# Nikhil-Kulkarni/RayTrace-miniapp

Measured on AMD Instinct MI355X. Metric: ray_steps_per_sec, higher is better.
Workload: dtype f32+f64

## Files before the change

### raytrace-miniapp_amd/csrc/rt_march.hip

```cpp
#pragma once
#include "rt_math.h"

#include <cfloat>

namespace rt {

enum : int { ST_IDLE = 0, ST_CELL = 1, ST_XSETUP = 2, ST_STEP = 3, ST_DONE = 4 };

typedef double f64x2 __attribute__((ext_vector_type(2)));
typedef float f32x4 __attribute__((ext_vector_type(4)));
typedef unsigned u32x4 __attribute__((ext_vector_type(4)));

__device__ __forceinline__ unsigned div_magic(unsigned x, unsigned mul, unsigned sh)
{
    return mul ? __umulhi(x, mul) >> sh : x;
}
__device__ __forceinline__ void grid_index(const DevRays &R, unsigned ridx, unsigned &i, unsigned &j, unsigned &k,
                                           unsigned &m)
{
    const unsigned ijkm = (unsigned) (R.first + (long long) ridx * R.stride);
    const unsigned q1   = div_magic(ijkm, R.div_mul[0], R.div_sh[0]);
    m                   = ijkm - q1 * (unsigned) R.ngb;
    const unsigned q2   = div_magic(q1, R.div_mul[1], R.div_sh[1]);
    k                   = q1 - q2 * (unsigned) R.nga;
    i                   = div_magic(q2, R.div_mul[2], R.div_sh[2]);
    j                   = q2 - i * (unsigned) R.ngy;
}

__device__ __forceinline__ void load_ray(const DevRays &R, unsigned ridx, rt_ray &ray, float &ta, float &tb,
                                         bool want_tan)
{
    if (R.list) {
        ray = R.list[ridx];
        if (want_tan) {
            ta = R.sxy[2 * (size_t) ridx];
            tb = R.sxy[2 * (size_t) ridx + 1];
        }
    } else {
        unsigned i, j, k, m;
        grid_index(R, ridx, i, j, k, m);
        ray.x      = (float) R.gx[i];
        ray.y      = (float) R.gy[j];
        ray.a      = (float) R.ga[k];
        ray.b      = (float) R.gb[m];
        if (want_tan) {
            ta = R.tan_a[k];
            tb = R.tan_b[m];
        }
    }
}

__device__ __attribute__((noinline)) float tan_wide(float x)
{
    if (!(fabsf(x) <= FLT_MAX))
        return x - x;
    return (float) tan((double) x);
}
__device__ __attribute__((noinline)) float atan_wide(float x)
{
    if (x != x)
        return x + x;
    if (!(fabsf(x) <= FLT_MAX))
        return copysignf(1.5707963705062866f, x);
    return (float) atan((double) x);
}

__device__ __attribute__((noinline)) float ktanf_flt32(float x, float y, int iy)
{
    const float T[13] = { 3.3333334327e-01f, 1.3333334029e-01f, 5.3968254477e-02f, 2.1869488060e-02f, 8.8632395491e-03f,
                          3.5920790397e-03f, 1.4562094584e-03f, 5.8804126456e-04f, 2.4646313977e-04f, 7.8179444245e-05f,
                          7.1407252108e-05f, -1.8558637748e-05f, 2.5907305826e-05f };
    const float pio4 = 7.8539812565e-01f, pio4lo = 3.7748947079e-08f;
    float z, r, v, w, s;
    const int hx = (int) __float_as_uint(x), ix = hx & 0x7fffffff;
    if (ix < 0x39000000) {
        if ((int) x == 0) {
            if ((ix | (iy + 1)) == 0)
                return 1.0f / fabsf(x);
            else if (iy == 1)
                return x;
            else
                return -1.0f / x;
        }
    }
    if (ix >= 0x3f2ca140) {
        if (hx < 0) {
            x = -x;
            y = -y;
        }
        z = pio4 - x;
        w = pio4lo - y;
        x = z + w;
        y = 0.0f;
        if (fabsf(x) < 0x1p-13f)
            return (1 - ((hx >> 30) & 2)) * iy * (1.0f - 2 * iy * x);
    }
    z = x * x;
    w = z * z;
    r = T[1] + w * (T[3] + w * (T[5] + w * (T[7] + w * (T[9] + w * T[11]))));
    v = z * (T[2] + w * (T[4] + w * (T[6] + w * (T[8] + w * (T[10] + w * T[12])))));
    s = z * x;
    r = y + z * (s * (r + v) + y);
    r += T[0] * s;
    w = x + r;
    if (ix >= 0x3f2ca140) {
        v = (float) iy;
        return (float) (1 - ((hx >> 30) & 2)) * (v - 2.0f * (x - (w * w / (w + v) - r)));
    }
    if (iy == 1)
        return w;
    float a, t;
    z = __uint_as_float(__float_as_uint(w) & 0xfffff000u);
    v = r - (z - x);
    t = a = -1.0f / w;
    t = __uint_as_float(__float_as_uint(t) & 0xfffff000u);
    s = 1.0f + t * z;
    return t + a * (s + t * v);
}
__device__ __attribute__((noinline)) float tanf_flt32_wide(float x)
{
    const float pio2_1 = 1.5707855225e+00f, pio2_1t = 1.0804334124e-05f, pio2_2 = 1.0804273188e-05f,
                pio2_2t = 6.0770999344e-11f;
    const int hx = (int) __float_as_uint(x), ix = hx & 0x7fffffff;
    if (ix <= 0x3f490fda)
        return ktanf_flt32(x, 0.0f, 1);
    float y0, y1, z;
    if (hx > 0) {
        z = x - pio2_1;
        if ((ix & 0xfffffff0) != 0x3fc90fd0) {
            y0 = z - pio2_1t;
            y1 = (z - y0) - pio2_1t;
        } else {
            z -= pio2_2;
            y0 = z - pio2_2t;
            y1 = (z - y0) - pio2_2t;
        }
    } else {
        z = x + pio2_1;
        if ((ix & 0xfffffff0) != 0x3fc90fd0) {
            y0 = z + pio2_1t;
            y1 = (z - y0) + pio2_1t;
        } else {
            z += pio2_2;
            y0 = z + pio2_2t;
            y1 = (z - y0) + pio2_2t;
        }
    }
    return ktanf_flt32(y0, y1, -1);
}

__device__ __forceinline__ float tanf_flt32_kernel(float x)
{
    const float ax = fabsf(x);
    if (ax < 0x1p-13f)
        return x;
    if (ax > 0.2f) {
        if (!(ax <= FLT_MAX))
            return x - x;
        return ax <= 1.375f ? tanf_flt32_wide(x) : tan_wide(x);
    }
    const float T0 = 3.3333334327e-01f, T1 = 1.3333334029e-01f, T2 = 5.3968254477e-02f, T3 = 2.1869488060e-02f,
                T4 = 8.8632395491e-03f, T5 = 3.5920790397e-03f, T6 = 1.4562094584e-03f, T7 = 5.8804126456e-04f,
                T8 = 2.4646313977e-04f, T9 = 7.8179444245e-05f, T10 = 7.1407252108e-05f, T11 = -1.8558637748e-05f,
                T12 = 2.5907305826e-05f;
    const float z = x * x;
    const float w = z * z;
    float r       = T1 + w * (T3 + w * (T5 + w * (T7 + w * (T9 + w * T11))));
    const float v = z * (T2 + w * (T4 + w * (T6 + w * (T8 + w * (T10 + w * T12)))));
    const float s = z * x;
    r             = 0.0f + z * (s * (r + v) + 0.0f);
    r += T0 * s;
    return x + r;
}

__device__ __forceinline__ float atanf_flt32_kernel(float x)
{
    const float ax = fabsf(x);
    if (ax < 0x1p-29f)
        return x;
    if (!(ax < 0.4375f))
        return atan_wide(x);
    const float A0 = 3.3333334327e-01f, A1 = -2.0000000298e-01f, A2 = 1.4285714924e-01f, A3 = -1.1111110449e-01f,
                A4 = 9.0908870101e-02f, A5 = -7.6918758452e-02f, A6 = 6.6610731184e-02f, A7 = -5.8335702866e-02f,
                A8 = 4.9768779427e-02f, A9 = -3.6531571299e-02f, A10 = 1.6285819933e-02f;
    const float z  = x * x;
    const float w  = z * z;
    const float s1 = z * (A0 + w * (A2 + w * (A4 + w * (A6 + w * (A8 + w * A10)))));
    const float s2 = w * (A1 + w * (A3 + w * (A5 + w * (A7 + w * A9))));
    return x - x * (s1 + s2);
}

extern "C" __global__ void __launch_bounds__(256) rt_seed_tab_kernel(const DevSeed sd, const DevRays R, double *sf,
                                                                     unsigned char *sin)
{
    const int n0 = R.ngx, n1 = R.ngy, n2 = R.nga, n3 = R.ngb;
    for (int t = (int) (blockIdx.x * blockDim.x + threadIdx.x); t < n0 + n1 + n2 + n3; t += (int) (gridDim.x * blockDim.x)) {
        int d           = t < n0 ? 0 : (t < n0 + n1 ? 1 : (t < n0 + n1 + n2 ? 2 : 3));
        const int i     = t - (d > 0 ? n0 : 0) - (d > 1 ? n1 : 0) - (d > 2 ? n2 : 0);
        const double *g = d == 0 ? R.gx : (d == 1 ? R.gy : (d == 2 ? R.ga : R.gb));
        const double v  = (double) (float) g[i];
        const bool in   = v >= sd.x[d][0] && v <= sd.x[d][sd.dim[d] - 1];
        sin[t]          = in ? 1 : 0;
        sf[t]           = in ? pchip_eval(sd.dim[d], sd.x[d], sd.f[d], v) : 0.0;
    }
}

__device__ __forceinline__ unsigned selftest_hash(unsigned x)
{
    x ^= x >> 16;
    x *= 0x7feb352du;
    x ^= x >> 15;
    x *= 0x846ca68bu;
    x ^= x >> 16;
    return x;
}
extern "C" __global__ void __launch_bounds__(256) rt_selftest_kernel(unsigned long long *counts)
{
    const unsigned lo = 0x3f700000u, hi = 0x3f880000u;
    const unsigned n_fast = hi - lo, n_other = 1u << 24;
    unsigned long long checked = 0, bad = 0;
    const unsigned long long tid = (unsigned long long) blockIdx.x * blockDim.x + threadIdx.x;
    const unsigned long long nth = (unsigned long long) gridDim.x * blockDim.x;
    for (unsigned long long t = tid; t < (unsigned long long) n_fast + n_other; t += nth) {
        const unsigned u = t < n_fast ? lo + (unsigned) t : (unsigned) (t - n_fast) << 8;
        float q          = __uint_as_float(u);
        const float a    = inv_norm(q);
        asm volatile("" : "+v"(q));
        const float b = 1.0f / sqrtf(q);
        checked++;
        if (__float_as_uint(a) != __float_as_uint(b) && !(a != a && b != b))
            bad++;
    }
    for (unsigned long long t = tid; t < (4ull << 23); t += nth) {
        float n       = __uint_as_float(0x3e800000u + (unsigned) t);
        const float a = fdiv_one_nr(n);
        asm volatile("" : "+v"(n));
        const float b = 1.0f / n;
        checked++;
        bad += __float_as_uint(a) != __float_as_uint(b) ? 1 : 0;
    }
    for (unsigned long long t = tid; t < (1ull << 28); t += nth) {
        const unsigned h0 = selftest_hash((unsigned) t * 2u + 1u), h1 = selftest_hash((unsigned) t * 2u + 0x9e3779b9u);
        const int ea = -84 + (int) (h0 % 84u), eb = -78 + (int) (h1 % 122u);
        if (ea - eb >= 96 || eb - ea >= 96 || ea - eb < -120)
            continue;
        float x = __uint_as_float(((unsigned) (ea + 127) << 23) | (selftest_hash(h0) & 0x7fffffu));
        float y = __uint_as_float(((unsigned) (eb + 127) << 23) | (selftest_hash(h1) & 0x7fffffu));
        const float a = fdiv_nr(x, y);
        asm volatile("" : "+v"(x), "+v"(y));
        const float b = x / y;
        checked++;
        bad += __float_as_uint(a) != __float_as_uint(b) ? 1 : 0;
    }
    if (tid == 0) {
        float inf = __uint_as_float(0x7f800000u), qnan = __uint_as_float(0x7fc00000u), big = 3.0e38f;
        asm volatile("" : "+v"(inf), "+v"(qnan), "+v"(big));
        const unsigned pio2 = 0x3fc90fdbu;
        const float t0 = tanf_flt32_kernel(inf), t1 = tanf_flt32_kernel(-inf), t2 = tanf_flt32_kernel(qnan), t3 = tan_wide(inf),
                    t4 = tan_wide(qnan), t5 = tanf_flt32_kernel(big);
        const float a0 = atanf_flt32_kernel(inf), a1 = atanf_flt32_kernel(-inf), a2 = atanf_flt32_kernel(qnan),
                    a3 = atanf_flt32_kernel(big), a4 = atanf_flt32_kernel(-big);
        checked += 11;
        bad += (t0 == t0) + (t1 == t1) + (t2 == t2) + (t3 == t3) + (t4 == t4) + (__float_as_uint(t5) == 0x7fc12345u);
        bad += (__float_as_uint(a0) != pio2) + (__float_as_uint(a1) != (pio2 | 0x80000000u)) + (a2 == a2) +
               (__float_as_uint(a3) != pio2) + (__float_as_uint(a4) != (pio2 | 0x80000000u));
    }
    atomicAdd(&counts[0], checked);
    atomicAdd(&counts[1], bad);
}

extern "C" __global__ void __launch_bounds__(256) rt_tan_kernel(const rt_ray *rays, unsigned long long n, float *sxy)
{
    unsigned long long i = (unsigned long long) blockIdx.x * blockDim.x + threadIdx.x;
    if (i < n) {
        rt_ray r       = rays[i];
        sxy[2 * i]     = tanf_flt32_kernel(1e-3f * r.a);
        sxy[2 * i + 1] = tanf_flt32_kernel(1e-3f * r.b);
    }
}

__device__ __forceinline__ int bisect_interval(const Interval *iv, int n, double v)
{
    int lo = 0, hi = n - 1;
    while (hi - lo != 1) {
        int mid = (hi + lo) / 2;
        if (iv[mid].hi >= v)
            hi = mid;
        else
            lo = mid;
    }
    return hi;
}
__device__ __forceinline__ int guess_interval(int n, float g0, float inv_h, float v)
{
    return (int) fminf(fmaxf((v - g0) * inv_h, 0.0f), (float) (n - 2)) + 1;
}

#ifdef RT_INSTRUMENT
__device__ unsigned short g_ray_iters[1u << 23];
#endif
#ifdef RT_WAVETIMES
__device__ unsigned long long g_wt[8];
__device__ unsigned long long g_wt_end[8192], g_wt_dry[8192];
constexpr int WT_TRACE = 64;
__device__ unsigned long long g_wt_trace[8192][WT_TRACE];
__device__ unsigned g_wt_blocks[8192][WT_TRACE][6];
#endif
struct TileList {
    unsigned *head;
    unsigned *next;
    unsigned *lnode;
    unsigned *nalloc;
    unsigned cap;
    unsigned *rem;
    unsigned *marching;
    unsigned n_waves;
    unsigned split;
    unsigned k_part;
};
constexpr unsigned TILE_NONE = 0xffffffffu;
constexpr unsigned TILE_PART_FLAG = 1u << 30, TILE_PART_SHIFT = 28, TILE_ID_MASK = (1u << TILE_PART_SHIFT) - 1u;
__device__ __forceinline__ unsigned tile_node(unsigned entry)
{
    return (entry & TILE_ID_MASK) * 4u + ((entry & TILE_PART_FLAG) ? (entry >> TILE_PART_SHIFT) & 3u : 0u);
}
#ifdef RT_WAVETIMES
__device__ unsigned long long g_wt_pub[8192][4];
__device__ unsigned long long g_wt_vm[8192];
#endif
constexpr unsigned TILE_REF_GLOBAL = 1u << 31;
__device__ __forceinline__ void tile_push(const TileList &T, unsigned tile)
{
    const unsigned id = __hip_atomic_fetch_add(T.nalloc, 1u, __ATOMIC_RELAXED, __HIP_MEMORY_SCOPE_WORKGROUP);
    unsigned old      = __hip_atomic_load(T.head, __ATOMIC_RELAXED, __HIP_MEMORY_SCOPE_WORKGROUP);
    if (id < T.cap) {
        __hip_atomic_store(&T.lnode[2u * id], tile, __ATOMIC_RELAXED, __HIP_MEMORY_SCOPE_WORKGROUP);
        for (;;) {
            __hip_atomic_store(&T.lnode[2u * id + 1u], old, __ATOMIC_RELAXED, __HIP_MEMORY_SCOPE_WORKGROUP);
            asm volatile("s_waitcnt lgkmcnt(0)" ::: "memory");
            if (__hip_atomic_compare_exchange_strong(T.head, &old, id, __ATOMIC_RELAXED, __ATOMIC_RELAXED, __HIP_MEMORY_SCOPE_WORKGROUP))
                return;
#ifdef RT_WAVETIMES
            g_wt_pub[(blockIdx.x * (blockDim.x >> 6) + (threadIdx.x >> 6)) & 8191u][2]++;
#endif
        }
    }
    tile |= TILE_REF_GLOBAL;
    for (;;) {
        __hip_atomic_store(&T.next[tile_node(tile & ~TILE_REF_GLOBAL)], old, __ATOMIC_RELAXED, __HIP_MEMORY_SCOPE_WORKGROUP);
        asm volatile("s_waitcnt vmcnt(0)" ::: "memory");
        if (__hip_atomic_compare_exchange_strong(T.head, &old, tile, __ATOMIC_RELAXED, __ATOMIC_RELAXED, __HIP_MEMORY_SCOPE_WORKGROUP))
            return;
#ifdef RT_WAVETIMES
        g_wt_pub[(blockIdx.x * (blockDim.x >> 6) + (threadIdx.x >> 6)) & 8191u][2]++;
#endif
    }
}
__device__ __forceinline__ void tile_publish(const TileList &T, unsigned tile)
{
    bool parts = T.split == 2u;
    if (T.split == 1u)
        parts = __hip_atomic_load(T.head, __ATOMIC_RELAXED, __HIP_MEMORY_SCOPE_WORKGROUP) == TILE_NONE &&
                __hip_atomic_load(T.marching, __ATOMIC_RELAXED, __HIP_MEMORY_SCOPE_WORKGROUP) * 8u <= T.n_waves;
    if (parts && T.k_part != 0u) {
        for (unsigned q = 0; q < 4u; q++)
            tile_push(T, tile | (q << TILE_PART_SHIFT) | TILE_PART_FLAG);
    } else {
        tile_push(T, tile);
    }
}
__device__ __forceinline__ unsigned tile_pop(const TileList &T)
{
    unsigned old = __hip_atomic_load(T.head, __ATOMIC_RELAXED, __HIP_MEMORY_SCOPE_WORKGROUP);
    while (old != TILE_NONE) {
        const unsigned nxt = (old & TILE_REF_GLOBAL)
                                 ? __hip_atomic_load(&T.next[tile_node(old & ~TILE_REF_GLOBAL)], __ATOMIC_RELAXED, __HIP_MEMORY_SCOPE_WORKGROUP)
                                 : __hip_atomic_load(&T.lnode[2u * old + 1u], __ATOMIC_RELAXED, __HIP_MEMORY_SCOPE_WORKGROUP);
        if (__hip_atomic_compare_exchange_strong(T.head, &old, nxt, __ATOMIC_RELAXED, __ATOMIC_RELAXED, __HIP_MEMORY_SCOPE_WORKGROUP))
            break;
    }
    if (old == TILE_NONE)
        return TILE_NONE;
    return (old & TILE_REF_GLOBAL) ? (old & ~TILE_REF_GLOBAL) : __hip_atomic_load(&T.lnode[2u * old], __ATOMIC_RELAXED, __HIP_MEMORY_SCOPE_WORKGROUP);
}

template <bool LDS_TAB> __device__ __forceinline__ void march_load_tables(const DevParams &P, unsigned char *lds_raw)
{
    if (LDS_TAB) {
        const uint4 *src = reinterpret_cast<const uint4 *>(P.blob);
        uint4 *dst       = reinterpret_cast<uint4 *>(lds_raw);
        const unsigned n16 = P.blob_bytes / 16, step = blockDim.x;
        for (unsigned i0 = threadIdx.x; i0 < n16; i0 += 8 * step) {
            uint4 v[8];
#pragma unroll
            for (int u = 0; u < 8; u++) {
                const unsigned i = i0 + (unsigned) u * step;
                v[u]             = src[i < n16 ? i : i0];
            }
#pragma unroll
            for (int u = 0; u < 8; u++) {
                const unsigned i = i0 + (unsigned) u * step;
                if (i < n16)
                    dst[i] = v[u];
            }
        }
        __syncthreads();
    }
}

template <bool LDS_TAB, bool BOUNDED, bool FUSED, int MODE = 0>
__device__ __forceinline__ void march_wave(const DevParams &P, unsigned char *lds_raw, const TileList done)
{
    const int lane        = lane_id();
    const int L           = P.L;
    const int S           = L * RT_N_SUB;
    const unsigned n_rays = P.ray_end;
    const bool backward   = MODE == 1 ? true : ((MODE == 2 || MODE == 3) ? false : P.method == 1);
    const bool use_emis   = MODE == 1 ? true : ((MODE == 2 || MODE == 4) ? false : P.use_emis != 0);
    const bool path_on    = MODE == 0 ? P.path_on != 0 : false;
    const unsigned CH     = P.chunk;
#ifndef RT_REFILL
#define RT_REFILL 8
#endif
    const int REFILL      = RT_REFILL;

    const unsigned char *tab = LDS_TAB ? lds_raw : P.blob;
    const BlobGain *hdr = reinterpret_cast<const BlobGain *>(tab);
    const unsigned lds_base = LDS_TAB ? (unsigned) (size_t) (__attribute__((address_space(3))) unsigned char *) lds_raw : 0u;

    static_assert(RT_N_SUB == 3, "sub-segment ends are tabulated for three sub-segments");
    float zs0 = (P.dz0 * (0.0f + 1.0f) / RT_N_SUB), zs1 = (P.dz0 * (1.0f + 1.0f) / RT_N_SUB),
          zs2 = (P.dz0 * (2.0f + 1.0f) / RT_N_SUB);
    asm volatile("" : "+v"(zs0), "+v"(zs1), "+v"(zs2));

    unsigned chunk_next = 0, chunk_end = 0;
    unsigned fetched_end = 0, slot_busy = 0, cur_slot = 0;
    unsigned cslot       = 0;
    bool more           = true;
    const unsigned n_launch_rays = n_rays - P.ray_begin;
    const unsigned n_chunks      = (n_launch_rays + CH - 1) / CH;
    unsigned shard = blockIdx.x & 7u, shards_seen_empty = 0;
    const unsigned n_main = n_chunks - (P.late_chunks < n_chunks ? P.late_chunks : 0u);
    const bool late_wave  = (unsigned) __builtin_amdgcn_readfirstlane((int) (threadIdx.x >> 6)) - P.late_first < P.late_waves;
    unsigned zone = 0;

    int st        = ST_IDLE;
    unsigned ridx = 0;
    int seg = 0, iz = 0, ii = 0;
    float z = 0.0f, z_stop = 0.0f;
    float px = 0, py = 0, pz = 0, sx = 0, sy = 0, sz = 1;
    float gacc = 0, eacc = 0;
    int cell_last = 0, sub = 0;
    unsigned char *recp = P.rec;
    unsigned lane12     = 0;
    BlobGain G    = hdr[1];
    unsigned steps = 0;
    bool escaped = false, mirror = false;
    unsigned any_bits = 0;
    int c00 = 0;
    float f00 = 1, f10 = 1, f01 = 1, f11 = 1;
    double dnx0 = 0, dnx1 = 0, dny0 = 0, dny1 = 0;
    f64x2 ix0 = { 0.0, 1.0 }, iy0 = { 0.0, 1.0 };
    f32x4 ix1 = { 1.0f, 0.0f, 0.0f, 0.0f }, iy1 = { 1.0f, 0.0f, 0.0f, 0.0f };
    float g0 = 0, E0 = 0;
    float dzrem = 0, zc = 0, path = 0;
    float rx = 0, ry = 0, rz = 0, n = 0, n0 = 0, gxn = 0, gyn = 0, lim2 = 0, dzcap = 0, hsum = 0;
    unsigned tot_steps = 0, tot_esc = 0, tot_rays = 0, tot_skip = 0;
#ifdef RT_INSTRUMENT
    Inst inst;
#endif

#if defined(RT_TIMEBLOCKS) || defined(RT_WAVEBLOCKS)
    unsigned long long tb_acc[6] = { 0, 0, 0, 0, 0, 0 }, tb_last = __builtin_readcyclecounter(), tb_iters = 0;
#endif
#ifdef RT_WAVETIMES
    const unsigned long long wt_start = __builtin_amdgcn_s_memrealtime();
    unsigned long long wt_dry = 0;
    unsigned wt_a_runs = 0, wt_b_runs = 0;
#endif
#ifdef RT_INSTRUMENT
    unsigned ray_iters = 0;
#endif
    unsigned spin = 0;
#if defined(RT_EXPRESS) || defined(RT_WAVETIMES)
    unsigned wave_iter = 0;
#endif
#ifdef RT_EXPRESS
    unsigned born = 0;
    bool old_wave = false;
    if (P.express_tail == 1u)
        __builtin_amdgcn_s_setprio(2);
#else
    constexpr bool old_wave = false;
#endif
    for (;;) {
        RT_MARK(5);
#ifdef RT_INSTRUMENT
        ray_iters += st != ST_IDLE ? 1u : 0u;
#endif
#ifdef RT_TIMEBLOCKS
        tb_iters++;
#endif
        unsigned long long idle2      = __ballot(st == ST_IDLE);
        const unsigned long long idle = idle2;
        const int n_idle              = (int) __popcll(idle);
#if defined(RT_EXPRESS) || defined(RT_WAVETIMES)
        wave_iter++;
#endif
#ifdef RT_WAVETIMES
        if ((wave_iter & 15u) == 0u) {
            const unsigned wid = blockIdx.x * (blockDim.x >> 6) + (threadIdx.x >> 6), smp = wave_iter >> 4;
            if (lane == 0 && wid < 8192u && smp < (unsigned) WT_TRACE) {
                g_wt_trace[wid][smp] = (__builtin_amdgcn_s_memrealtime() & 0xffffffffffull) | ((unsigned long long) (WAVE - n_idle) << 40) |
                                       ((unsigned long long) wt_a_runs << 48) | ((unsigned long long) wt_b_runs << 56);
                g_wt_trace[wid][0] = smp;
#ifdef RT_WAVEBLOCKS
                for (int b = 0; b < 6; b++)
                    g_wt_blocks[wid][smp][b] = (unsigned) tb_acc[b];
#endif
            }
#ifdef RT_WAVEBLOCKS
            for (int b = 0; b < 6; b++)
                tb_acc[b] = 0;
#endif
            wt_a_runs = wt_b_runs = 0;
        }
#endif
#ifdef RT_EXPRESS
        if (P.express_age != 0u && (wave_iter & 3u) == 0u) {
            const bool o = __ballot(st != ST_IDLE && wave_iter - born > P.express_age) != 0ull;
            if (o != old_wave) {
                old_wave = o;
                if (o)
                    __builtin_amdgcn_s_setprio(3);
                else
                    __builtin_amdgcn_s_setprio(0);
            }
        }
#endif
        if (!BOUNDED) {
            if (((++spin) & 0xfffu) == 0u && spin >= P.spin_limit) {
                spin = 0;
                if (st != ST_IDLE) {
                    escaped = true;
                    sx = sy = sz = 0.0f;
                    st           = ST_CELL;
                }
            }
        }
        if (more && (n_idle >= REFILL)) {
            const int rank = (int) __builtin_amdgcn_mbcnt_hi((unsigned) (idle >> 32),
                                                             __builtin_amdgcn_mbcnt_lo((unsigned) idle, 0u));
            int need = n_idle, off = 0;
            bool got = false;
            while (need > 0) {
                if (chunk_next == chunk_end && !(FUSED && chunk_next != fetched_end)) {
#ifdef RT_EXPRESS
                    if (old_wave && P.express_hold != 0u)
                        break;
#endif
                    unsigned c = 0;
#ifdef RT_MARCH_ONE_COUNTER
                    if (lane == 0)
                        c = atomicAdd(&P.ctl->next_tile[P.launch_id][0][0], 1u);
                    c = (unsigned) __builtin_amdgcn_readfirstlane((int) c);
                    shards_seen_empty = 7;
#else
                    if (lane == 0)
                        c = atomicAdd(&P.ctl->next_tile[P.launch_id][shard][zone * 8u], 1u);
                    c = (unsigned) __builtin_amdgcn_readfirstlane((int) c) * 8u + shard + zone * n_main;
#endif
                    if (c >= (zone ? n_chunks : n_main)) {
                        if (++shards_seen_empty == 8) {
                            if (zone == 0u && late_wave && n_main < n_chunks) {
                                zone              = 1u;
                                shards_seen_empty = 0;
                                continue;
                            }
                            more = false;
#ifdef RT_EXPRESS
                            if (P.express_tail == 2u)
                                __builtin_amdgcn_s_setprio(3);
#endif
#ifdef RT_WAVETIMES
                            wt_dry = __builtin_amdgcn_s_memrealtime();
#endif
                            break;
                        }
                        shard = (shard + 1) & 7u;
                        continue;
                    }
                    chunk_next = P.ray_begin + c * CH;
                    chunk_end  = (n_rays - chunk_next < CH) ? n_rays : chunk_next + CH;
                    if (FUSED) {
                        fetched_end = chunk_end;
                        chunk_end   = chunk_next;
                    }
                }
                if (FUSED && chunk_next == chunk_end) {
#ifndef RT_FUSED_PUBLISH_WAVE
                    const unsigned in_use = lane < 32 ? __hip_atomic_load(&done.rem[lane], __ATOMIC_RELAXED, __HIP_MEMORY_SCOPE_WAVEFRONT) : 1u;
                    slot_busy             = ~(unsigned) __ballot(lane < 32 && in_use == 0u);
#endif
                    const int fs = __builtin_ffs((int) ~slot_busy) - 1;
                    if (fs < 0)
                        break;
                    chunk_end = fetched_end - chunk_next < (unsigned) WAVE ? fetched_end : chunk_next + (unsigned) WAVE;
                    cur_slot  = (unsigned) fs;
                    slot_busy |= 1u << fs;
                    if (lane == 0)
                        __hip_atomic_store(&done.rem[fs], chunk_end - chunk_next, __ATOMIC_RELAXED, __HIP_MEMORY_SCOPE_WAVEFRONT);
                }
                int avail = (int) (chunk_end - chunk_next);
                int take  = avail < need ? avail : need;
                if (st == ST_IDLE && !got && rank >= off && rank < off + take) {
                    ridx = chunk_next + (unsigned) (rank - off);
                    got  = true;
                    if (FUSED)
                        cslot = cur_slot;
                }
                chunk_next += (unsigned) take;
                need -= take;
                off += take;
            }
            if (!BOUNDED && __ballot(got) != 0ull)
                spin = 0;
            if (got) {
                rt_ray ray;
                float ta = 0, tb = 0;
                load_ray(P.rays, ridx, ray, ta, tb, true);
                px = ray.x;
                py = ray.y;
                pz = 0.0f;
                sx = ta;
                sy = tb;
                sz = 1.0f;
                if (backward) {
                    sx = -sx;
                    sy = -sy;
                    sz = -sz;
                }
                renormalise(sx, sy, sz);
                const BlobGain G0 = hdr[backward ? P.N - 1 : 1];
                const float dsum  = sx + sy + sz;
                const bool wild   = ((px != px) | (py != py) | (dsum != dsum)) &
                                  !((px < G0.lo_x) | (px > G0.hi_x) | (py < G0.lo_y) | (py > G0.hi_y));
                if (path_on) {
                    float *pp = P.path + (size_t) ridx * 3 * (size_t) (S + 1) + 3 * (size_t) (backward ? S : 0);
                    pp[0]     = px;
                    pp[1]     = py;
                }
                recp      = P.rec + rec_slot_off(ridx, backward ? S - 1 : 0, P.rec_stride);
                lane12    = (ridx & 63u) * 12u;
                seg       = 0;
                iz        = 0;
                ii        = backward ? P.N - 1 : 1;
                G         = G0;
                z         = 0.0f;
                z_stop    = zs0;
                gacc      = 0.0f;
                eacc      = 0.0f;
                cell_last = 0;
                steps     = 0;
                escaped   = wild;
                sx        = wild ? 0.0f : sx;
                sy        = wild ? 0.0f : sy;
                sz        = wild ? 0.0f : sz;
                any_bits  = P.no_skip;
                sub       = 0;
                st        = ST_CELL;
#ifdef RT_EXPRESS
                born      = wave_iter;
#endif
            }
            idle2 = __ballot(st == ST_IDLE);
        }
        if (idle2 == ~0ull) {
            if (!more)
                break;
        } else {

        RT_MARK(0);
        const unsigned long long want_a = __ballot(st == ST_CELL);
        int park_at = (int) P.park;
        if (!more || old_wave || (int) P.park > 12 || REFILL > 8) {
            const int n_live = WAVE - (int) __popcll(idle2);
            const int fifth  = (n_live * 13 + 63) >> 6;
            park_at          = fifth < (int) P.park ? fifth : (int) P.park;
#ifdef RT_EXPRESS
            if (old_wave && P.express_park != 0u)
                park_at = (n_live * (int) P.express_park + 63) >> 6;
#endif
        }
        const bool do_a = (int) __popcll(want_a) >= park_at || (~(idle2 | want_a)) == 0ull;
#ifdef RT_FUSED_PUBLISH_WAVE
        bool last_of_tile = false;
#endif
#ifdef RT_WAVETIMES
        wt_a_runs += (do_a && want_a != 0ull) ? 1u : 0u;
        wt_b_runs += __ballot(st == ST_XSETUP) != 0ull ? 1u : 0u;
#endif
        if (do_a && st == ST_CELL) {
            bool in_seg        = !escaped & (z < 0.995f * z_stop);
            if (!in_seg) {
#ifndef RT_ABL_NOSTORE
                *reinterpret_cast<RecSlot *>(recp) = RecSlot{ gacc, eacc, cell_last };
#endif
                recp += backward ? -(int) REC_SLOT_ROW : (int) REC_SLOT_ROW;
                any_bits |= (__float_as_uint(gacc) | __float_as_uint(eacc)) & 0x7fffffffu;
                if (path_on) {
                    float *pp = P.path + (size_t) ridx * 3 * (size_t) (S + 1);
                    for (int zz = iz; zz < (escaped ? RT_N_SUB : iz + 1); zz++) {
                        const int idx = RT_N_SUB * (ii - 1) + (backward ? RT_N_SUB - zz - 1 : zz + 1);
                        pp[3 * idx]     = px;
                        pp[3 * idx + 1] = py;
                    }
                }
                gacc      = 0.0f;
                eacc      = 0.0f;
                cell_last = 0;
                sub++;
                const bool wrap = iz == RT_N_SUB - 1;
                const bool fin  = escaped | (sub == S);
                iz              = wrap ? 0 : iz + 1;
                z               = wrap ? 0.0f : z;
                st              = fin ? ST_DONE : ST_CELL;
                if (wrap & !fin) {
                    seg++;
                    ii = backward ? P.N - seg - 1 : seg + 1;
                    G  = hdr[ii];
                }
                z_stop = iz == 0 ? zs0 : (iz == 1 ? zs1 : zs2);
                in_seg = !fin & (z < 0.995f * z_stop);
            }
            RT_MARK(1);
            if ((st == ST_CELL) & in_seg) {
                if ((px < G.lo_x) | (px > G.hi_x) | (py < G.lo_y) | (py > G.hi_y) | (sz * sz <= 0.01f)) {
                    escaped = true;
                } else {
                    mirror              = G.mirror_y != 0;
                    const Interval *ivx = reinterpret_cast<const Interval *>(tab + G.off_ix);
                    const Interval *ivy = reinterpret_cast<const Interval *>(tab + G.off_iy);
                    f64x2 tx, ty;
                    u32x4 q00, q10, q01, q11;
                    auto gather = [&](int k1, int k2, int c) {
                        const unsigned ox = (unsigned) G.off_ix + (unsigned) k1 * (unsigned) sizeof(Interval);
                        const unsigned oy = (unsigned) G.off_iy + (unsigned) k2 * (unsigned) sizeof(Interval);
                        const unsigned oa = (unsigned) G.off_node + (unsigned) c * (unsigned) sizeof(Node);
                        const unsigned ob = oa + (unsigned) G.Nx * (unsigned) sizeof(Node);
                        if (LDS_TAB) {
                            asm volatile("ds_read_b128 %0, %10\n\t"
                                         "ds_read_b128 %1, %10 offset:16\n\t"
                                         "ds_read_b128 %2, %10 offset:32\n\t"
                                         "ds_read_b128 %3, %11\n\t"
                                         "ds_read_b128 %4, %11 offset:16\n\t"
                                         "ds_read_b128 %5, %11 offset:32\n\t"
                                         "ds_read_b128 %6, %12\n\t"
                                         "ds_read_b128 %7, %12 offset:16\n\t"
                                         "ds_read_b128 %8, %13\n\t"
                                         "ds_read_b128 %9, %13 offset:16\n\t"
                                         "s_waitcnt lgkmcnt(0)"
                                         : "=&v"(ix0), "=&v"(ix1), "=&v"(tx), "=&v"(iy0), "=&v"(iy1), "=&v"(ty), "=&v"(q00), "=&v"(q10),
                                           "=&v"(q01), "=&v"(q11)
                                         : "v"(lds_base + ox), "v"(lds_base + oy), "v"(lds_base + oa), "v"(lds_base + ob));
                        } else {
                            const unsigned char *t = tab;
                            ix0 = *reinterpret_cast<const f64x2 *>(t + ox);
                            ix1 = *reinterpret_cast<const f32x4 *>(t + ox + 16);
                            tx  = *reinterpret_cast<const f64x2 *>(t + ox + 32);
                            iy0 = *reinterpret_cast<const f64x2 *>(t + oy);
                            iy1 = *reinterpret_cast<const f32x4 *>(t + oy + 16);
                            ty  = *reinterpret_cast<const f64x2 *>(t + oy + 32);
                            q00 = *reinterpret_cast<const u32x4 *>(t + oa);
                            q10 = *reinterpret_cast<const u32x4 *>(t + oa + 16);
                            q01 = *reinterpret_cast<const u32x4 *>(t + ob);
                            q11 = *reinterpret_cast<const u32x4 *>(t + ob + 16);
                        }
                    };
                    auto node_n = [](const u32x4 &q) { return __hiloint2double((int) q.y, (int) q.x); };
                    const float ya      = mirror ? fabsf(py) : py;
                    const double pxd = (double) px, yad = (double) ya;
                    int k1     = guess_interval(G.Nx, G.x0f, G.inv_hxf, px);
                    int k2     = guess_interval(G.Ny, G.y0f, G.inv_hyf, ya);
                    c00        = (k1 - 1) + (k2 - 1) * G.Nx;
                    gather(k1, k2, c00);
                    const bool ok = ((k1 == 1) | (ix0.x < pxd)) & ((k1 == G.Nx - 1) | (tx.x >= pxd)) &
                                    ((k2 == 1) | (iy0.x < yad)) & ((k2 == G.Ny - 1) | (ty.x >= yad));
                    if (!ok) {
                        k1  = bisect_interval(ivx, G.Nx, pxd);
                        k2  = bisect_interval(ivy, G.Ny, yad);
                        c00 = (k1 - 1) + (k2 - 1) * G.Nx;
                        gather(k1, k2, c00);
                    }
                    const double n00 = node_n(q00), n10 = node_n(q10), n01 = node_n(q01), n11 = node_n(q11);
                    f00       = (float) n00;
                    f10       = (float) n10;
                    f01       = (float) n01;
                    f11       = (float) n11;
                    dnx0      = n10 - n00;
                    dnx1      = n11 - n01;
                    dny0      = n01 - n00;
                    dny1      = n11 - n10;
                    const float u = (float) div_by_recip<true>(pxd - ix0.x, tx.x - ix0.x, tx.y);
                    const float v = (float) div_by_recip<true>(yad - iy0.x, ty.x - iy0.x, ty.y);
                    g0            = lerp2(u, v, __uint_as_float(q00.z), __uint_as_float(q10.z), __uint_as_float(q01.z),
                                          __uint_as_float(q11.z));
                    E0            = 0.0f;
                    if (use_emis) {
                        E0 = lerp2(u, v, __uint_as_float(q00.w), __uint_as_float(q10.w), __uint_as_float(q01.w),
                                   __uint_as_float(q11.w));
                        E0 = E0 >= 0 ? E0 : 0.0f;
                    }
                    pz    = 0.0f;
                    zc    = 0.0f;
                    path  = 0.0f;
                    dzrem = z_stop - z;
                    if ((px > ix1.y) & (px < ix1.z) & (ya > iy1.y) & (ya < iy1.z) & (dzrem > 0.0f)) {
                        st = ST_XSETUP;
                    } else {
                        z += fabsf(pz);
                        gacc += g0 * path;
                        eacc += E0 * path;
                        cell_last = c00;
                        steps++;
                        RT_TICK(2);
                    }
                }
            }
            RT_MARK(2);
            if (st == ST_DONE) {
                unsigned fl = F_VALID;
                if (escaped)
                    fl |= F_ESCAPED;
                if (use_emis && any_bits == 0u)
                    fl |= F_SKIP;
                RecMeta m;
                m.px          = px;
                m.py          = py;
                m.sx          = sx;
                m.sy          = sy;
                m.sz          = sz;
                m.flags_steps = fl | ((unsigned) sub << REC_NDONE_SHIFT) |
                                ((steps < 0xfffffu ? steps : 0xfffffu) << REC_STEPS_SHIFT);
                unsigned char *metap = recp + (int) REC_SLOT_ROW * (backward ? sub + 1 : S - sub) + lane12;
#ifndef RT_ABL_NOMETA
                *reinterpret_cast<RecMeta *>(metap) = m;
#else
                if (m.px == 1234.5f)
                    *reinterpret_cast<RecMeta *>(metap) = m;
#endif
#ifdef RT_INSTRUMENT
                if (ridx < (1u << 23))
                    g_ray_iters[ridx] = (unsigned short) (ray_iters < 65535u ? ray_iters : 65535u);
                ray_iters = 0;
#endif
                tot_steps += steps;
                tot_esc += escaped ? 1u : 0u;
                tot_skip += (fl & F_SKIP) ? 1u : 0u;
                tot_rays++;
                st = ST_IDLE;
#ifdef RT_FUSED_PUBLISH_WAVE
                if (FUSED)
                    last_of_tile = __hip_atomic_fetch_add(&done.rem[cslot], 0xffffffffu, __ATOMIC_RELAXED, __HIP_MEMORY_SCOPE_WAVEFRONT) == 1u;
#else
                if (FUSED) {
                    if (__hip_atomic_fetch_add(&done.rem[cslot], 0xffffffffu, __ATOMIC_RELAXED, __HIP_MEMORY_SCOPE_WAVEFRONT) == 1u) {
                        asm volatile("s_waitcnt vmcnt(0)" ::: "memory");
                        tile_publish(done, ridx >> 6);
                    }
                }
#endif
            }
        }
#ifdef RT_FUSED_PUBLISH_WAVE
        if (FUSED) {
            unsigned long long lm = __ballot(last_of_tile);
            if (lm != 0ull) {
#ifdef RT_WAVETIMES
                const unsigned long long vm0 = __builtin_amdgcn_s_memrealtime();
#endif
                asm volatile("s_waitcnt vmcnt(0)" ::: "memory");
#ifdef RT_WAVETIMES
                if (lane == 0)
                    g_wt_vm[(blockIdx.x * (blockDim.x >> 6) + (threadIdx.x >> 6)) & 8191u] += __builtin_amdgcn_s_memrealtime() - vm0;
#endif
                do {
                    const int l0 = (int) __ffsll((long long) lm) - 1;
                    lm &= lm - 1ull;
#ifdef RT_WAVETIMES
                    const unsigned long long pub0 = __builtin_amdgcn_s_memrealtime();
#endif
                    if (lane == l0)
                        tile_publish(done, ridx >> 6);
#ifdef RT_WAVETIMES
                    if (lane == l0) {
                        const unsigned long long dt = __builtin_amdgcn_s_memrealtime() - pub0;
                        unsigned long long *q = g_wt_pub[(blockIdx.x * (blockDim.x >> 6) + (threadIdx.x >> 6)) & 8191u];
                        q[0] += dt;
                        q[1] += 1;
                        q[3] = dt > q[3] ? dt : q[3];
                    }
#endif
                    slot_busy &= ~(1u << (unsigned) __builtin_amdgcn_readlane((int) cslot, l0));
                } while (lm != 0ull);
            }
        }
#endif
        RT_MARK(3);
        if (st == ST_XSETUP) {
            const float ya   = mirror ? fabsf(py) : py;
            const double dwx = (double) ix1.x, dwy = (double) iy1.x;
            const double xc0 = ix0.x, yc0 = iy0.x, rwx = ix0.y, rwy = iy0.y;
            const float u    = (float) div_by_recip<true>((double) px - xc0, dwx, rwx);
            const float v    = (float) div_by_recip<true>((double) ya - yc0, dwy, rwy);
            n0  = lerp2(u, v, f00, f10, f01, f11);
            gxn = (float) (div_by_recip<true>((1.0 - (double) v) * dnx0, dwx, rwx) +
                           div_by_recip<true>((double) v * dnx1, dwx, rwx));
            gyn = (float) (div_by_recip<true>((1.0 - (double) u) * dny0, dwy, rwy) +
                           div_by_recip<true>((double) u * dny1, dwy, rwy));
            if (mirror && py < 0)
                gyn = -gyn;
            lim2  = dzrem - zc;
            dzcap = P.c_cap * lim2;
            rx    = 0.0f;
            ry    = 0.0f;
            rz    = 0.0f;
            n     = n0;
            hsum  = 0.0f;
            st    = ST_STEP;
            RT_TICK(1);
        }

        RT_MARK(4);
        if (st == ST_STEP) {
            const float lim0 = 0.1f * ix1.x, lim1 = 0.1f * iy1.x;
            bool run;
            {
                n        = n0 + rx * gxn + ry * gyn;
#ifdef RT_ABL_FASTDIV
#define RT_FDIV(a, b) ((a) * __builtin_amdgcn_rcpf(b))
#else
#define RT_FDIV(a, b) ((a) / (b))
#endif
                const float rn = BOUNDED ? fdiv_one_nr(n) : RT_FDIV(1.0f, n);
                float a0 = sx * gxn + sy * gyn + 1e-12f;
                float t  = BOUNDED ? fmaf(fmaf(-n, a0 * rn, a0), rn, a0 * rn) : div_by_recip_signed(a0, n, rn);
                float qx = div_by_recip_signed(gxn, n, rn);
                float qy = div_by_recip_signed(gyn, n, rn);
#ifndef RT_ABL_NOGUARD
                if (__ballot(fminf(fminf(fabsf(a0), fabsf(gxn)), fabsf(gyn)) < 1e-29f) != 0ull) {
#ifdef RT_INSTRUMENT
                    if (lane == (int) __ffsll((long long) __ballot(1)) - 1)
                        atomicAdd(&g_inst[6], 1ull);
#endif
                    if (fabsf(a0) < 1e-29f && a0 != 0.0f) {
                        asm volatile("" : "+v"(a0));
                        t = a0 / n;
                    }
                    if (fabsf(gxn) < 1e-29f && gxn != 0.0f) {
                        float g = gxn;
                        asm volatile("" : "+v"(g));
                        qx = g / n;
                    }
                    if (fabsf(gyn) < 1e-29f && gyn != 0.0f) {
                        float g = gyn;
                        asm volatile("" : "+v"(g));
                        qy = g / n;
                    }
                }
#endif
                float fx = qx - sx * t;
                float fy = qy - sy * t;
                float fz = -sz * t;
                float h;
                if (BOUNDED) {
                    const float h1 = fdiv_nr(P.c_h1, fabsf(t));
                    const float h2 = fdiv_nr(1.0001f * (lim2 - fabsf(rz)), fabsf(sz));
                    const float h3 = fdiv_nr(P.c_h3 * (fabsf(sx) + 5e-4f), (fabsf(fx) + 1e-8f));
                    const float h4 = fdiv_nr(P.c_h3 * (fabsf(sy) + 5e-4f), (fabsf(fy) + 1e-8f));
                    h = fmin_nan_drop(fmin_nan_drop(h1, dzcap), fmin_nan_drop(h2, fmin_nan_drop(h3, h4)));
                } else {
                    h        = RT_FDIV(P.c_h1, fabsf(t));
                    h        = h < dzcap ? h : dzcap;
                    float h2 = RT_FDIV(1.0001f * (lim2 - fabsf(rz)), fabsf(sz));
                    float h3 = RT_FDIV(P.c_h3 * (fabsf(sx) + 5e-4f), (fabsf(fx) + 1e-8f));
                    float h4 = RT_FDIV(P.c_h3 * (fabsf(sy) + 5e-4f), (fabsf(fy) + 1e-8f));
                    h        = h < h2 ? h : h2;
                    h        = h < h3 ? h : h3;
                    h        = h < h4 ? h : h4;
                }
                float ht = h * t;
                const float R3 = 1.0f / 3.0f, R6 = 1.0f / 6.0f, R12 = 1.0f / 12.0f;
                float c1 = 0.5f * h * h * (1.0f - div_by_recip<true>(ht, 3.0f, R3) + div_by_recip<true>(ht * ht, 12.0f, R12));
                rx += sx * h + c1 * fx;
                ry += sy * h + c1 * fy;
                rz += sz * h + c1 * fz;
                float c2 = h * (1.0f - 0.5f * ht + div_by_recip<true>(ht * ht, 6.0f, R6));
                sx += c2 * fx;
                sy += c2 * fy;
                sz += c2 * fz;
                renormalise(sx, sy, sz);
                hsum += h;
                RT_TICK(0);
                run = (fabsf(rx) < lim0) & (fabsf(ry) < lim1) & (fabsf(rz) < lim2) & (fabsf(n - n0) < 0.05f);
            }
            if (!run) {
                path += hsum;
                px += rx;
                py += ry;
                pz += rz;
                zc += fabsf(rz);
                const float ya = mirror ? fabsf(py) : py;
                if ((px > ix1.y) & (px < ix1.z) & (ya > iy1.y) & (ya < iy1.z) & ((double) zc < 0.999 * (double) dzrem)) {
                    st = ST_XSETUP;
                } else {
                    z += fabsf(pz);
                    gacc += g0 * path;
                    eacc += E0 * path;
                    cell_last = c00;
                    steps++;
                    RT_TICK(2);
                    st = ST_CELL;
                }
            }
        }
        }
    }
#ifdef RT_EXPRESS
    if (P.express_age != 0u || P.express_tail != 0u)
        __builtin_amdgcn_s_setprio(0);
#endif

#ifdef RT_WAVETIMES
    if (lane == 0) {
        const unsigned long long wt_end = __builtin_amdgcn_s_memrealtime();
        atomicMin(&g_wt[0], wt_start);
        atomicMax(&g_wt[1], wt_start);
        const unsigned w = atomicAdd((unsigned *) &g_wt[6], 1u);
        if (w < 8192)
            g_wt_end[w] = wt_end | ((unsigned long long) (threadIdx.x >> 6) << 56), g_wt_dry[w] = wt_dry;
    }
#endif
    {
        unsigned s = wave_sum_u32(tot_steps), e = wave_sum_u32(tot_esc);
        unsigned k = wave_sum_u32(tot_skip), r = wave_sum_u32(tot_rays);
#ifndef RT_ABL_NOTOTALS
        if (lane == 0) {
            atomicAdd(&P.ctl->cell_steps, (unsigned long long) s);
            atomicAdd(&P.ctl->n_escaped, (unsigned long long) e);
            atomicAdd(&P.ctl->n_skipped, (unsigned long long) k);
            atomicAdd(&P.ctl->n_rays, (unsigned long long) r);
        }
#else
        if (lane == 0 && s + e + k + r == 0xffffffffu)
            atomicAdd(&P.ctl->cell_steps, 1ull);
#endif
#ifdef RT_TIMEBLOCKS
        if (lane == 0) {
            for (int i = 0; i < 6; i++)
                atomicAdd(&g_inst[i], tb_acc[i]);
            atomicAdd(&g_inst[7], tb_iters);
        }
#endif
#ifdef RT_INSTRUMENT
        for (int i = 0; i < 3; i++) {
            unsigned tw = wave_sum_u32(inst.w[i]), ta = wave_sum_u32(inst.a[i]);
            if (lane == 0) {
                atomicAdd(&g_inst[2 * i], (unsigned long long) tw);
                atomicAdd(&g_inst[2 * i + 1], (unsigned long long) ta);
            }
        }
#endif
    }
}

template <bool LDS_TAB, bool BOUNDED, int MODE = 0>
__global__ void __launch_bounds__(LDS_TAB ? 1024 : 256) rt_march_kernel(const DevParams P)
{
    extern __shared__ __align__(16) unsigned char lds_raw[];
    march_load_tables<LDS_TAB>(P, lds_raw);
    march_wave<LDS_TAB, BOUNDED, false, MODE>(P, lds_raw, TileList{ nullptr, nullptr, nullptr, nullptr, 0u, nullptr, nullptr, 0u, 0u, 0u });
}

}
```

Measured before the change: 29.40 billion.

## Precompute ray start state per tile and hand it to lanes via bpermute

```diff
diff --git a/raytrace-miniapp_amd/csrc/rt_march.hip b/raytrace-miniapp_amd/csrc/rt_march.hip
--- a/raytrace-miniapp_amd/csrc/rt_march.hip
+++ b/raytrace-miniapp_amd/csrc/rt_march.hip
@@ -423,6 +423,11 @@
 #define RT_REFILL 8
 #endif
     const int REFILL      = RT_REFILL;
+#ifdef RT_NO_TILE_START
+    constexpr bool TILE_START = false;
+#else
+    constexpr bool TILE_START = FUSED;
+#endif
 
     const unsigned char *tab = LDS_TAB ? lds_raw : P.blob;
     const BlobGain *hdr = reinterpret_cast<const BlobGain *>(tab);
@@ -466,6 +471,28 @@
     float dzrem = 0, zc = 0, path = 0;
     float rx = 0, ry = 0, rz = 0, n = 0, n0 = 0, gxn = 0, gyn = 0, lim2 = 0, dzcap = 0, hsum = 0;
     unsigned tot_steps = 0, tot_esc = 0, tot_rays = 0, tot_skip = 0;
+    float bank_px = 0, bank_py = 0, bank_sx = 0, bank_sy = 0, bank_sz = 0;
+    unsigned long long bank_wild = 0ull;
+    auto start_state = [&](const unsigned r, float &qx, float &qy, float &ux, float &uy, float &uz) {
+        rt_ray ray;
+        float ta = 0, tb = 0;
+        load_ray(P.rays, r, ray, ta, tb, true);
+        qx = ray.x;
+        qy = ray.y;
+        ux = ta;
+        uy = tb;
+        uz = 1.0f;
+        if (backward) {
+            ux = -ux;
+            uy = -uy;
+            uz = -uz;
+        }
+        renormalise(ux, uy, uz);
+        const BlobGain &G0 = hdr[backward ? P.N - 1 : 1];
+        const float dsum   = ux + uy + uz;
+        return (bool) (((qx != qx) | (qy != qy) | (dsum != dsum)) &
+                       !((qx < G0.lo_x) | (qx > G0.hi_x) | (qy < G0.lo_y) | (qy > G0.hi_y)));
+    };
 #ifdef RT_INSTRUMENT
     Inst inst;
 #endif
@@ -610,15 +637,40 @@
                     slot_busy |= 1u << fs;
                     if (lane == 0)
                         __hip_atomic_store(&done.rem[fs], chunk_end - chunk_next, __ATOMIC_RELAXED, __HIP_MEMORY_SCOPE_WAVEFRONT);
+                    if (TILE_START) {
+                        const unsigned r = chunk_next + (unsigned) lane;
+                        const bool wild  = start_state(r < chunk_end ? r : chunk_end - 1u, bank_px, bank_py, bank_sx, bank_sy, bank_sz);
+                        bank_sx          = wild ? 0.0f : bank_sx;
+                        bank_sy          = wild ? 0.0f : bank_sy;
+                        bank_sz          = wild ? 0.0f : bank_sz;
+                        bank_wild        = __ballot(wild);
+                    }
                 }
                 int avail = (int) (chunk_end - chunk_next);
                 int take  = avail < need ? avail : need;
-                if (st == ST_IDLE && !got && rank >= off && rank < off + take) {
+                const bool mine = st == ST_IDLE && !got && rank >= off && rank < off + take;
+                if (mine) {
                     ridx = chunk_next + (unsigned) (rank - off);
                     got  = true;
                     if (FUSED)
                         cslot = cur_slot;
                 }
+                if (TILE_START) {
+                    const int src  = (int) ((chunk_next + (unsigned) (rank - off)) & 63u) << 2;
+                    const float vx = __int_as_float(__builtin_amdgcn_ds_bpermute(src, __float_as_int(bank_px)));
+                    const float vy = __int_as_float(__builtin_amdgcn_ds_bpermute(src, __float_as_int(bank_py)));
+                    const float wx = __int_as_float(__builtin_amdgcn_ds_bpermute(src, __float_as_int(bank_sx)));
+                    const float wy = __int_as_float(__builtin_amdgcn_ds_bpermute(src, __float_as_int(bank_sy)));
+                    const float wz = __int_as_float(__builtin_amdgcn_ds_bpermute(src, __float_as_int(bank_sz)));
+                    if (mine) {
+                        px      = vx;
+                        py      = vy;
+                        sx      = wx;
+                        sy      = wy;
+                        sz      = wz;
+                        escaped = ((bank_wild >> (ridx & 63u)) & 1ull) != 0ull;
+                    }
+                }
                 chunk_next += (unsigned) take;
                 need -= take;
                 off += take;
@@ -626,25 +678,14 @@
             if (!BOUNDED && __ballot(got) != 0ull)
                 spin = 0;
             if (got) {
-                rt_ray ray;
-                float ta = 0, tb = 0;
-                load_ray(P.rays, ridx, ray, ta, tb, true);
-                px = ray.x;
-                py = ray.y;
+                if (!TILE_START) {
+                    const bool wild = start_state(ridx, px, py, sx, sy, sz);
+                    escaped         = wild;
+                    sx              = wild ? 0.0f : sx;
+                    sy              = wild ? 0.0f : sy;
+                    sz              = wild ? 0.0f : sz;
+                }
                 pz = 0.0f;
-                sx = ta;
-                sy = tb;
-                sz = 1.0f;
-                if (backward) {
-                    sx = -sx;
-                    sy = -sy;
-                    sz = -sz;
-                }
-                renormalise(sx, sy, sz);
-                const BlobGain G0 = hdr[backward ? P.N - 1 : 1];
-                const float dsum  = sx + sy + sz;
-                const bool wild   = ((px != px) | (py != py) | (dsum != dsum)) &
-                                  !((px < G0.lo_x) | (px > G0.hi_x) | (py < G0.lo_y) | (py > G0.hi_y));
                 if (path_on) {
                     float *pp = P.path + (size_t) ridx * 3 * (size_t) (S + 1) + 3 * (size_t) (backward ? S : 0);
                     pp[0]     = px;
@@ -655,17 +696,13 @@
                 seg       = 0;
                 iz        = 0;
                 ii        = backward ? P.N - 1 : 1;
-                G         = G0;
+                G         = hdr[backward ? P.N - 1 : 1];
                 z         = 0.0f;
                 z_stop    = zs0;
                 gacc      = 0.0f;
                 eacc      = 0.0f;
                 cell_last = 0;
                 steps     = 0;
-                escaped   = wild;
-                sx        = wild ? 0.0f : sx;
-                sy        = wild ? 0.0f : sy;
-                sz        = wild ? 0.0f : sz;
                 any_bits  = P.no_skip;
                 sub       = 0;
                 st        = ST_CELL;
```

After: 29.21 billion. No clear change (-0.7%).

## Stage ray loads cooperatively per chunk and distribute via cross-lane permutes

Applied to the files above, without the earlier changes.

```diff
diff --git a/raytrace-miniapp_amd/csrc/rt_march.hip b/raytrace-miniapp_amd/csrc/rt_march.hip
--- a/raytrace-miniapp_amd/csrc/rt_march.hip
+++ b/raytrace-miniapp_amd/csrc/rt_march.hip
@@ -482,6 +482,34 @@
     unsigned ray_iters = 0;
 #endif
     unsigned spin = 0;
+    float g_px = 0, g_py = 0, g_sx = 0, g_sy = 0, g_sz = 0;
+    unsigned stage_base = 0, stage_end = 0;
+    auto stage_rays = [&](unsigned base, unsigned end) {
+        const unsigned r = base + (unsigned) lane;
+        if (r < end) {
+            rt_ray ray;
+            float ta = 0, tb = 0;
+            load_ray(P.rays, r, ray, ta, tb, true);
+            g_px = ray.x;
+            g_py = ray.y;
+            g_sx = ta;
+            g_sy = tb;
+            g_sz = 1.0f;
+            if (backward) {
+                g_sx = -g_sx;
+                g_sy = -g_sy;
+                g_sz = -g_sz;
+            }
+            renormalise(g_sx, g_sy, g_sz);
+            const BlobGain &G0 = hdr[backward ? P.N - 1 : 1];
+            const float dsum   = g_sx + g_sy + g_sz;
+            const bool wild    = ((g_px != g_px) | (g_py != g_py) | (dsum != dsum)) &
+                              !((g_px < G0.lo_x) | (g_px > G0.hi_x) | (g_py < G0.lo_y) | (g_py > G0.hi_y));
+            g_sx = wild ? 0.0f : g_sx;
+            g_sy = wild ? 0.0f : g_sy;
+            g_sz = wild ? 0.0f : g_sz;
+        }
+    };
 #if defined(RT_EXPRESS) || defined(RT_WAVETIMES)
     unsigned wave_iter = 0;
 #endif
@@ -610,15 +638,36 @@
                     slot_busy |= 1u << fs;
                     if (lane == 0)
                         __hip_atomic_store(&done.rem[fs], chunk_end - chunk_next, __ATOMIC_RELAXED, __HIP_MEMORY_SCOPE_WAVEFRONT);
-                }
-                int avail = (int) (chunk_end - chunk_next);
+                    stage_rays(chunk_next, chunk_end);
+                } else if (!FUSED && chunk_next - stage_base >= stage_end - stage_base) {
+                    stage_base = chunk_next;
+                    stage_end  = chunk_end - chunk_next < (unsigned) WAVE ? chunk_end : chunk_next + (unsigned) WAVE;
+                    stage_rays(stage_base, stage_end);
+                }
+                int avail = (int) ((FUSED ? chunk_end : stage_end) - chunk_next);
                 int take  = avail < need ? avail : need;
-                if (st == ST_IDLE && !got && rank >= off && rank < off + take) {
+                const bool now = st == ST_IDLE && !got && rank >= off && rank < off + take;
+                if (now) {
                     ridx = chunk_next + (unsigned) (rank - off);
                     got  = true;
                     if (FUSED)
                         cslot = cur_slot;
                 }
+                {
+                    const int src = (now ? (int) (ridx - (FUSED ? (chunk_next & ~(unsigned) (WAVE - 1)) : stage_base)) : lane) << 2;
+                    const float t0 = __int_as_float(__builtin_amdgcn_ds_bpermute(src, __float_as_int(g_px)));
+                    const float t1 = __int_as_float(__builtin_amdgcn_ds_bpermute(src, __float_as_int(g_py)));
+                    const float t2 = __int_as_float(__builtin_amdgcn_ds_bpermute(src, __float_as_int(g_sx)));
+                    const float t3 = __int_as_float(__builtin_amdgcn_ds_bpermute(src, __float_as_int(g_sy)));
+                    const float t4 = __int_as_float(__builtin_amdgcn_ds_bpermute(src, __float_as_int(g_sz)));
+                    if (now) {
+                        px = t0;
+                        py = t1;
+                        sx = t2;
+                        sy = t3;
+                        sz = t4;
+                    }
+                }
                 chunk_next += (unsigned) take;
                 need -= take;
                 off += take;
@@ -626,25 +675,9 @@
             if (!BOUNDED && __ballot(got) != 0ull)
                 spin = 0;
             if (got) {
-                rt_ray ray;
-                float ta = 0, tb = 0;
-                load_ray(P.rays, ridx, ray, ta, tb, true);
-                px = ray.x;
-                py = ray.y;
                 pz = 0.0f;
-                sx = ta;
-                sy = tb;
-                sz = 1.0f;
-                if (backward) {
-                    sx = -sx;
-                    sy = -sy;
-                    sz = -sz;
-                }
-                renormalise(sx, sy, sz);
                 const BlobGain G0 = hdr[backward ? P.N - 1 : 1];
-                const float dsum  = sx + sy + sz;
-                const bool wild   = ((px != px) | (py != py) | (dsum != dsum)) &
-                                  !((px < G0.lo_x) | (px > G0.hi_x) | (py < G0.lo_y) | (py > G0.hi_y));
+                const bool wild = sz == 0.0f;
                 if (path_on) {
                     float *pp = P.path + (size_t) ridx * 3 * (size_t) (S + 1) + 3 * (size_t) (backward ? S : 0);
                     pp[0]     = px;
@@ -663,9 +696,6 @@
                 cell_last = 0;
                 steps     = 0;
                 escaped   = wild;
-                sx        = wild ? 0.0f : sx;
-                sy        = wild ? 0.0f : sy;
-                sz        = wild ? 0.0f : sz;
                 any_bits  = P.no_skip;
                 sub       = 0;
                 st        = ST_CELL;
```

Result: no change. 29.45 billion before, 29.59 billion after, median of 6 (+0.5%).
